# lazear/sage

Measured on AMD Instinct MI355X. Metric: spectra/sec (whole node), fragment-index search-and-score, human tryptic narrow search, higher is better.
Workload: dtype f32

## Files before the change

sage_amd/csrc/core.h:

```cpp
#pragma once
#include <stdint.h>

#if defined(__HIPCC__)
#define SAGE_HD __host__ __device__ __forceinline__
#else
#define SAGE_HD inline
#endif

namespace sagecore {

constexpr float PROTON = 1.0072764f;
constexpr float NEUTRON = 1.00335f;

struct Tol {
    int kind;
    float lo, hi;
};

SAGE_HD void tol_bounds(const Tol& t, float center, float& out_lo, float& out_hi) {
    if (t.kind == 0) {
        float dlo = center * t.lo / 1000000.0f;
        float dhi = center * t.hi / 1000000.0f;
        out_lo = center + dlo;
        out_hi = center + dhi;
// ... 537 lines not shown
constexpr uint32_t PLUT_BINS = 256;
SAGE_HD float peak_lut_width(float top) {
    uint32_t bits;
    __builtin_memcpy(&bits, &top, 4);
    const uint32_t e = (bits >> 23) & 0xFFu;
    uint32_t we = (bits >> 31) || e < 134u ? 127u : e - 7u;
    we = we > 227u ? 227u : we;
    const uint32_t wb = we << 23;
    float w;
    __builtin_memcpy(&w, &wb, 4);
    return w;
}
SAGE_HD float pow2_reciprocal(float w) {
    uint32_t bits;
    __builtin_memcpy(&bits, &w, 4);
    bits = 0x7F000000u - bits;
    float r;
    __builtin_memcpy(&r, &bits, 4);
    return r;
}
SAGE_HD uint32_t peak_lut_entry(const float* pm, uint32_t P, uint32_t b, float w) {
    if (b == 0) return 0;
    const int32_t edge = order_key((float)b * w);
    uint32_t lo = 0, hi = P;
    while (lo < hi) {
        const uint32_t mid = (lo + hi) >> 1;
        if (order_key(pm[mid]) < edge) lo = mid + 1; else hi = mid;
    }
    return lo;
}
SAGE_HD int select_peak_lut(const float* pm, const float* pi, uint32_t P, const uint32_t* plut, float inv_w, float lo, float hi) {
    float fb = __builtin_floorf(lo * inv_w);
    fb = fb > 0.0f ? fb : 0.0f;
    const uint32_t bin = fb < (float)(PLUT_BINS - 1) ? (uint32_t)fb : PLUT_BINS - 1;
    int best = -1;
    float max_int = 0.0f;
    for (uint32_t a = plut[bin]; a < P; a += 2) {
        const float m0 = pm[a], m1 = pm[a + 1 < P ? a + 1 : a];
        if (m0 >= lo && m0 <= hi) {
            const float it = pi[a];
            if (it >= max_int) { max_int = it; best = (int)a; }
        }
        if (a + 1 < P && m1 >= lo && m1 <= hi) {
            const float it = pi[a + 1];
            if (it >= max_int) { max_int = it; best = (int)(a + 1); }
        }
        if (m0 > hi || m1 > hi || !(hi == hi)) break;
    }
    return best;
}

SAGE_HD uint32_t wpp_step(uint32_t span) { return span / 65u + 1u; }

#ifndef SAGE_PBM_LOG2_BITS
#define SAGE_PBM_LOG2_BITS 15
#endif
#ifndef SAGE_PBM_LOG2_INV_W
#define SAGE_PBM_LOG2_INV_W 4
#endif
constexpr uint32_t PBM_BITS = 1u << SAGE_PBM_LOG2_BITS, PBM_WORDS = PBM_BITS / 32;
constexpr float PBM_INV_W = (float)(1u << SAGE_PBM_LOG2_INV_W);
constexpr float PBM_MAX_D = 4.0f;
SAGE_HD uint32_t pbm_index(float ion) {
#if defined(__HIP_DEVICE_COMPILE__)
    const float f = ion * PBM_INV_W;
    uint32_t x;
    asm("v_cvt_u32_f32 %0, %1" : "=v"(x) : "v"(f));
    return x;
#else
    const float f = ion * PBM_INV_W;
    return f >= 4294967296.0f ? 0xFFFFFFFFu : f > 0.0f ? (uint32_t)f : 0u;
#endif
}
SAGE_HD uint32_t pbm_bin_c1(uint32_t x) { return x & (PBM_BITS - 1u); }
SAGE_HD uint32_t pbm_bin_c2(uint32_t x) { return (x >> 1) & (PBM_BITS - 1u); }
SAGE_HD uint32_t pbm_bin_c3(uint32_t x) { return (uint32_t)(((uint64_t)x * 0xAAAAAAABull) >> 33) & (PBM_BITS - 1u); }
struct PbmReach {
    float a, b;
};
SAGE_HD PbmReach pbm_reach_of(const Tol& t) {
    const float tmax = __builtin_fmaxf(__builtin_fabsf(t.lo), __builtin_fabsf(t.hi));
    const float rel = t.kind == 0 ? tmax * 1.0e-6f : t.kind == 1 ? tmax * 1.0e-2f : 0.0f;
    PbmReach r{-1.0f, 0.0f};
    if (!(tmax == tmax) || !(tmax < 1.0e30f) || !(rel < 0.25f)) return r;
    r.a = (rel / (1.0f - rel)) * 1.0002f + (1.0f / 1048576.0f);
    r.b = (t.kind == 2 ? tmax * 1.0002f : 0.0f) + (1.0f / 1048576.0f);
    return r;
}
SAGE_HD bool pbm_peak_reach(const PbmReach& r, float m, float& D) {
    D = __builtin_fmaf(m, r.a, r.b);
    return r.a >= 0.0f && m >= 0.0f && m < 8388608.0f && D <= PBM_MAX_D;
}
SAGE_HD void pbm_peak_span(float m, float D, uint32_t& b0, uint32_t& b1) {
    const float f0 = (m - D) * PBM_INV_W, f1 = (m + D) * PBM_INV_W;
    b0 = f0 > 0.0f ? (uint32_t)f0 : 0u;
    b1 = f1 > 0.0f ? (uint32_t)f1 : 0u;
}

SAGE_HD uint32_t flat_octets(uint32_t n_here) { return (n_here + 7u) >> 3; }
SAGE_HD uint32_t flat_item_k(uint32_t t, uint32_t owner_start) { return t - owner_start; }
SAGE_HD uint64_t flat_item_base(uint64_t chunk_at, uint32_t owner_start) { return chunk_at - 8ull * owner_start; }
SAGE_HD uint64_t flat_item_ion(uint64_t item_base, uint32_t t) { return item_base + 8ull * t; }
SAGE_HD uint32_t flat_stride(uint32_t total) { return (total + 3u) & ~3u; }
SAGE_HD uint32_t flat_area_bytes(uint32_t total, uint32_t ncharges) { return flat_stride(total) * ncharges + 12u; }
#ifndef SAGE_FLAT_MARGIN
#define SAGE_FLAT_MARGIN 1
// ... 15 lines not shown
```

sage_amd/csrc/kernels.hip:

```cpp
#include <hip/hip_runtime.h>

#include <type_traits>

#include "crlog.h"
#include "device_types.h"

using namespace sagecore;

namespace sagehip {

namespace {

#ifndef SAGE_PRELIM_WAVES
#define SAGE_PRELIM_WAVES 5
#endif
#ifndef SAGE_RESCORE_WAVES
#define SAGE_RESCORE_WAVES 5
#endif
#ifndef SAGE_NARROW_WAVES
#define SAGE_NARROW_WAVES 5
#endif
#ifndef SAGE_PROBE_PER_LANE
#define SAGE_PROBE_PER_LANE 2
#endif
#ifndef SAGE_PROBE_CELLS
#define SAGE_PROBE_CELLS 4
#endif
#ifndef SAGE_TILE8_CELLS
#define SAGE_TILE8_CELLS 2
#endif
#ifndef SAGE_MARK_BLOCKS8
#define SAGE_MARK_BLOCKS8 96
#endif
#ifndef SAGE_MARK_BLOCKS16
#define SAGE_MARK_BLOCKS16 40
#endif
#ifndef SAGE_COOP_MIN_HITS
#define SAGE_COOP_MIN_HITS 12
#endif
#ifndef SAGE_COOP_MAX_LANES
#define SAGE_COOP_MAX_LANES 2
#endif
#ifndef SAGE_CNT_MODE
#define SAGE_CNT_MODE 0
#endif
#ifndef SAGE_SCAN_SKIP
#define SAGE_SCAN_SKIP 1
#endif
#if SAGE_NARROW_WAVES
#define SAGE_NARROW_WAVES_ATTR __attribute__((amdgpu_waves_per_eu(SAGE_NARROW_WAVES, SAGE_NARROW_WAVES)))
#else
#define SAGE_NARROW_WAVES_ATTR
#endif
#if SAGE_PRELIM_WAVES
#define SAGE_PRELIM_WAVES_ATTR __attribute__((amdgpu_waves_per_eu(SAGE_PRELIM_WAVES, SAGE_PRELIM_WAVES)))
#else
#define SAGE_PRELIM_WAVES_ATTR
#endif
#if SAGE_RESCORE_WAVES
#define SAGE_RESCORE_WAVES_ATTR __attribute__((amdgpu_waves_per_eu(SAGE_RESCORE_WAVES, SAGE_RESCORE_WAVES)))
#else
#define SAGE_RESCORE_WAVES_ATTR
#endif

constexpr uint32_t WAVE = 64;
constexpr uint32_t NO_WINDOW = 0xFFFFFFFFu;
constexpr uint32_t FAST_TIE_WORDS = PBM_WORDS + PLUT_BINS;
constexpr uint32_t CNT_ROW_HEADER = 4;
constexpr uint32_t PROBE_BATCH_WORDS = SAGE_PROBE_PER_LANE * 64;
constexpr uint32_t PROBE_TCS_WORDS = PROBE_BATCH_WORDS <= 64 ? 64 : PROBE_BATCH_WORDS <= 128 ? 128 : PROBE_BATCH_WORDS <= 256 ? 256 : 512;
constexpr uint32_t PROBE_TABLE_WORDS = 4 * PROBE_BATCH_WORDS + PROBE_TCS_WORDS;

enum { DBG_PRUNE_CAND = 0, DBG_PRUNE_ITEMS = 1, DBG_PRUNE_EARLY = 2, DBG_PRUNE_MIXED = 3 };
enum { DBG_FILTER_FLAT_CHUNKS = 4, DBG_FILTER_FLAT_TRIPS = 5, DBG_FILTER_FLAT_WOULD = 6, DBG_FILTER_LANE_TRIPS = 7 };
enum { DBG_HEAVY_CHUNKS = 8, DBG_HEAVY_ITEMS = 9 };
enum { DBG_HEAVY_ONE_TRIP = 10, DBG_HEAVY_PER_CHARGE = 11 };
enum { DBG_NARROW_LUT = 26, DBG_NARROW_CELLS = 27, DBG_RESCORE = 28, DBG_TILE_LUT = 29, DBG_TILE_CELLS = 30, DBG_TILE_CAND = 31 };
struct PhaseClock {
    unsigned long long* slot;
    long long t;
    __device__ __forceinline__ void bytes(int which, unsigned long long n) {
        if (slot) atomicAdd(&slot[which - row_base], n);
    }
    int row_base;
    unsigned long long* prune;
    uint32_t pruned_here;
    __device__ __forceinline__ void pruned(uint64_t lanes, uint32_t items) {
        if (slot && lanes) {
            pruned_here += (uint32_t)__popcll(lanes);
            if ((threadIdx.x & 63u) == 0) {
                atomicAdd(&prune[DBG_PRUNE_CAND], (unsigned long long)__popcll(lanes));
                atomicAdd(&prune[DBG_PRUNE_ITEMS], (unsigned long long)items);
            }
        }
    }
    __device__ __forceinline__ void filter_trips(bool flat, uint32_t flat_trips, uint32_t lane_trips) {
        if (slot && (threadIdx.x & 63u) == 0) {
            if (flat) {
                atomicAdd(&prune[DBG_FILTER_FLAT_CHUNKS], 1ull);
                atomicAdd(&prune[DBG_FILTER_FLAT_TRIPS], (unsigned long long)flat_trips);
                atomicAdd(&prune[DBG_FILTER_FLAT_WOULD], (unsigned long long)lane_trips);
            } else {
                atomicAdd(&prune[DBG_FILTER_LANE_TRIPS], (unsigned long long)lane_trips);
            }
        }
    }
    __device__ __forceinline__ void heavy(uint32_t items) {
        if (slot && (threadIdx.x & 63u) == 0) {
            atomicAdd(&prune[DBG_HEAVY_CHUNKS], 1ull);
            atomicAdd(&prune[DBG_HEAVY_ITEMS], (unsigned long long)items);
        }
    }
    __device__ __forceinline__ void heavy_route(bool one_trip) {
        if (slot && (threadIdx.x & 63u) == 0) atomicAdd(&prune[one_trip ? DBG_HEAVY_ONE_TRIP : DBG_HEAVY_PER_CHARGE], 1ull);
    }
    __device__ __forceinline__ void prune_outcome(bool left_early, bool any_pass) {
        if (slot && (threadIdx.x & 63u) == 0) {
            if (left_early) atomicAdd(&prune[DBG_PRUNE_EARLY], 1ull);
            else if (any_pass && pruned_here) atomicAdd(&prune[DBG_PRUNE_MIXED], 1ull);
        }
        pruned_here = 0;
    }
// ... 315 lines not shown
            uint32_t rank = 0;
            if (i < nst)
                for (uint32_t j = 0; j < nst; j++) {
                    const uint64_t o = c.items[j];
                    rank += (o > keep_v[q]) || (o == keep_v[q] && j < i);
                }
            keep_r[q] = i < nst ? rank : 0xFFFFFFFFu;
        }
        wave_sync();
#pragma unroll
        for (uint32_t q = 0; q < 4; q++)
            if (keep_r[q] < k) c.items[keep_r[q]] = keep_v[q];
        for (uint32_t i = nst + lane; i < k; i += WAVE) c.items[i] = PRESCORE_EMPTY;
        wave_sync();
    }
    c.stored = k;
    c.len = k;
}

__device__ __forceinline__ void lh_build(uint64_t* a, uint32_t k) {
    wave_sync();
    if (lane_id() == 0) heap_build(a, k);
    wave_sync();
}
__device__ __forceinline__ void lh_offer_batch(uint64_t* a, uint32_t k, uint64_t v, bool has) {
    if (!k) return;
    uint64_t mask = __ballot(has && v > a[0]);
    if (!mask) return;
    while (mask) {
        const uint32_t bit = (uint32_t)__ffsll((long long)mask) - 1;
        mask &= mask - 1;
        const uint64_t o = lane_value(v, bit);
        if (lane_id() == 0) heap_offer(a, k, o);
    }
    wave_sync();
}
__device__ __forceinline__ void ulist_trim_big(UList& c, uint32_t report_psms) {
    const uint32_t lane = lane_id();
    const uint32_t k = trim_k(c.len, report_psms);
    if (c.len > k) {
        lh_build(c.items, k);
        for (uint32_t base = k; base < c.stored; base += WAVE) {
            const bool has = base + lane < c.stored;
            lh_offer_batch(c.items, k, has ? c.items[base + lane] : 0ull, has);
        }
    }
    c.stored = k;
    c.len = k;
}

struct PrelimLds {
    float* win_lo;
    float* win_hi;
    uint64_t* listA;
    uint64_t* listB;
    uint64_t* heap;
    uint32_t* ptab;
    uint32_t* cnt;
};

__device__ __forceinline__ PrelimLds carve_prelim(unsigned char* smem, const DevScorer& sc, const DevBatchView& b, unsigned char* big = nullptr) {
    PrelimLds l;
    size_t off = 0;
    const bool fold = sc.min_isotope_err != sc.max_isotope_err;
    if (big) {
        l.listA = (uint64_t*)big;
        l.listB = l.listA + (fold ? (size_t)sc.list_cap : 0);
        l.heap = l.listB + sc.list_cap;
    } else {
        l.listA = (uint64_t*)(smem + off); off += fold ? (size_t)sc.list_cap * 8 : 0;
        l.listB = (uint64_t*)(smem + off); off += (size_t)sc.list_cap * 8;
        l.heap = (uint64_t*)(smem + off); off += (size_t)sc.kmax * 8;
    }
    const size_t win = b.probe ? (size_t)b.pcap * 4 : (size_t)b.fzcap * b.pcap * 4;
    l.win_lo = (float*)(smem + off); off += win;
    l.win_hi = (float*)(smem + off); off += b.probe ? 0 : win;
    off = (off + 3) & ~(size_t)3;
    l.ptab = (uint32_t*)(smem + off); off += b.probe ? (size_t)PROBE_TABLE_WORDS * 4 : 0;
    l.cnt = (uint32_t*)(smem + off);
    return l;
}

__host__ __device__ inline size_t prelim_big_bytes(const DevScorer& sc) {
    const bool fold = sc.min_isotope_err != sc.max_isotope_err;
    return (size_t)sc.list_cap * (fold ? 16 : 8) + (size_t)sc.kmax * 8;
}
__host__ __device__ inline size_t prelim_layout_bytes(const DevScorer& sc, const DevBatchView& b, bool huge = false) {
    size_t n = (huge ? 0 : prelim_big_bytes(sc)) +
               (b.probe ? (size_t)b.pcap * 4 + 4 + (size_t)PROBE_TABLE_WORDS * 4 : (size_t)b.fzcap * b.pcap * 8);
    n += ((size_t)sc.wcap / 2 + 1) * 4;
    return (n + 15) & ~(size_t)15;
}

struct SpecInfo {
    uint64_t p0;
    uint32_t P, z0, z1, nfz_max;
    float mzp;
    Tol iso_tol;
    Window win;
    bool has_win;
};
__device__ __forceinline__ SpecInfo load_spec(const DevScorer& sc, const DevBatchView& b, uint32_t spec) {
    SpecInfo s;
    s.win = Window{0u, 0u, 0u, 0u};
    s.has_win = false;
    s.p0 = uni64(b.peak_off[spec]);
    s.P = (uint32_t)(uni64(b.peak_off[spec + 1]) - s.p0);
    const uint32_t zraw = uni(b.precursor_charge[spec]);
    if (sc.wide_window || zraw == 0 || sc.override_precursor_charge) {
        s.z0 = sc.min_precursor_charge;
        s.z1 = sc.max_precursor_charge;
    } else {
        s.z0 = s.z1 = zraw;
    }
    s.nfz_max = 0;
    for (uint32_t z = s.z0; z <= s.z1; z++) {
        const uint32_t m = max_fragment_charge(sc.max_fragment_charge, z) - 1;
        s.nfz_max = m > s.nfz_max ? m : s.nfz_max;
    }
    if (s.nfz_max > b.fzcap) s.nfz_max = b.fzcap;
    s.mzp = unif(b.precursor_mz[spec]) - PROTON;
    s.iso_tol.kind = 2;
    s.iso_tol.lo = -2.4f;
    s.iso_tol.hi = 2.4f;
    if (b.isolation_lo && b.isolation_hi) {
        const float a = unif(b.isolation_lo[spec]), c = unif(b.isolation_hi[spec]);
        if (a == a && c == c) {
            s.iso_tol.lo = a;
            s.iso_tol.hi = c;
            if (b.iso_kind) s.iso_tol.kind = (int32_t)uni(b.iso_kind[spec]);
        }
    }
    return s;
}

__device__ __forceinline__ SpecInfo load_spec_sched(const DevScorer& sc, const DevBatchView& b, uint32_t pos, uint32_t& spec) {
    const uint4* __restrict__ rec = b.sched + (size_t)b.sched_stride * pos;
    const uint4 r0 = rec[0], r1 = rec[1];
    uint4 r2 = make_uint4(NO_WINDOW, 0u, 0u, 0u);
    if (b.sched_win) r2 = rec[2];
    spec = uni(r0.x);
    SpecInfo s;
// ... 119 lines not shown
    }
    wave_sync();
    ulist_append(target, lane < nsel ? sel[lane] : PRESCORE_EMPTY, k, kmax);
    wave_sync();
    return true;
}

constexpr uint32_t PROBE_PER_LANE = SAGE_PROBE_PER_LANE;
constexpr uint32_t PROBE_BATCH = PROBE_PER_LANE * 64;
constexpr uint32_t PROBE_CELLS = SAGE_PROBE_CELLS;
static_assert(PROBE_BATCH == PROBE_BATCH_WORDS && PROBE_BATCH <= 512, "the run table's layout (carve_prelim) is the kernel's");
static_assert(PROBE_TCS_WORDS - PROBE_BATCH <= WAVE, "one sentinel per lane pads the run starts");
struct PrelimKernargs {
    DevDbView db;
    DevScorer sc;
    DevBatchView b;
    DevWork w;
};
#define SAGE_LOAD_TOL(t) Tol{(t).kind, (t).lo, (t).hi}
template <class K>
struct ArgRef {
    const DevDbView& db_;
    const DevScorer& sc_;
    const DevBatchView& b_;
    __device__ __forceinline__ ArgRef(const DevDbView& d, const DevScorer& s, const DevBatchView& b) : db_(d), sc_(s), b_(b) {}
    __device__ __forceinline__ void refresh() {}
    __device__ __forceinline__ const DevDbView& db() const { return db_; }
    __device__ __forceinline__ const DevScorer& sc() const { return sc_; }
    __device__ __forceinline__ const DevBatchView& b() const { return b_; }
};
template <>
struct ArgRef<PrelimKernargs> {
    typedef const __attribute__((address_space(4))) PrelimKernargs* Segment;
    Segment ka;
    __device__ __forceinline__ ArgRef(const DevDbView&, const DevScorer&, const DevBatchView&)
        : ka((Segment)__builtin_amdgcn_kernarg_segment_ptr()) {}
    __device__ __forceinline__ void refresh() {
        ka = (Segment)__builtin_amdgcn_kernarg_segment_ptr();
        asm volatile("" : "+s"(ka));
    }
    __device__ __forceinline__ const __attribute__((address_space(4))) DevDbView& db() const { return ka->db; }
    __device__ __forceinline__ const __attribute__((address_space(4))) DevScorer& sc() const { return ka->sc; }
    __device__ __forceinline__ const __attribute__((address_space(4))) DevBatchView& b() const { return ka->b; }
};

struct PrelimResult {
    uint32_t stored;
    uint32_t matched, scored;
    bool ok;
    bool deferred;
    bool untrimmed;
    uint32_t q_left, q_potential;
};
template <bool PROBE, bool BIGK = false, class KA = void, class PC>
__device__ __forceinline__ PrelimResult prelim_spectrum(const DevDbView& db_, const DevScorer& sc_, const DevBatchView& b_, const PrelimLds& L,
                                                        const SpecInfo& si, const bool exact, PC& pc) {
    const uint32_t lane = lane_id();
    ArgRef<KA> av(db_, sc_, b_);
    av.refresh();
    Counters cnt;
    cnt.p = L.cnt;
    PrelimResult res{0u, 0u, 0u, true, false, true, 0u, 0u};
    {
        const uint32_t P = si.P, nfz_max = si.nfz_max;
        const float* __restrict__ masses = av.b().masses + si.p0;
        const uint32_t pcap = av.b().pcap;
        const Tol ftol0 = SAGE_LOAD_TOL(av.sc().fragment_tol);

        float pk0 = 0.f, pk1 = 0.f, pk2 = 0.f;
        Window q_first{0u, 0u, 0u, 0u};
        bool have_first = false;
        int iso_first = 0;
        if (PROBE) {
            if (lane < P) pk0 = masses[lane];
            if (lane + WAVE < P) pk1 = masses[lane + WAVE];
            if (lane + 2 * WAVE < P) pk2 = masses[lane + 2 * WAVE];
        }
        if (si.z0 <= si.z1) {
            const bool fold0 = av.sc().min_isotope_err != av.sc().max_isotope_err;
            iso_first = fold0 ? av.sc().min_isotope_err : 0;
            if (si.has_win && !(av.sc().dbg_flags & 65536u)) {
                q_first = si.win;
                have_first = true;
            } else if (PROBE) {
                const float precursor_mass = si.mzp * (float)si.z0;
                const Tol ptol = av.sc().wide_window ? tol_scaled(si.iso_tol, (float)si.z0) : SAGE_LOAD_TOL(av.sc().precursor_tol);
                const float center = precursor_mass - (float)iso_first * NEUTRON;
                q_first = query_window<true>(av.db().pep_mono, av.db().np, ptol, center, av.db().pep_lut, av.db().pep_lut_bins, av.db().pep_lut_inv_w);
                have_first = true;
            }
        }
        if (PROBE) {
            if (lane < P) L.win_lo[lane] = pk0;
            if (lane + WAVE < P) L.win_lo[lane + WAVE] = pk1;
            if (lane + 2 * WAVE < P) L.win_lo[lane + 2 * WAVE] = pk2;
        }
        for (uint32_t i = PROBE ? lane + 3 * WAVE : lane; i < P; i += WAVE) {
            const float m = masses[i];
            if (PROBE) {
                L.win_lo[i] = m;
                continue;
            }
            for (uint32_t fz = 1; fz <= nfz_max; fz++) {
                float lo, hi;
                tol_bounds(ftol0, m * (float)fz, lo, hi);
                L.win_lo[(size_t)(fz - 1) * pcap + i] = lo;
                L.win_hi[(size_t)(fz - 1) * pcap + i] = hi;
            }
        }
        __syncthreads();
        if (pc.slot && lane == 0) pc.bytes(DBG_NARROW_CELLS, 4ull * P);
        bool sorted_ok = true;
        uint32_t ptop = 0;
        if (!PROBE) {
            bool mono_ok = true;
            for (uint32_t fz = 0; fz < nfz_max; fz++) {
                const float* wl = L.win_lo + (size_t)fz * pcap;
                const float* wh = L.win_hi + (size_t)fz * pcap;
                for (uint32_t i = lane; i < P; i += WAVE) {
                    mono_ok = mono_ok && (wl[i] <= wh[i]);
                    if (i > 0) mono_ok = mono_ok && (wl[i - 1] <= wl[i]) && (wh[i - 1] <= wh[i]);
                }
            }
            sorted_ok = __ballot(!mono_ok) == 0ull;
            ptop = pow2_floor(P);
        }
        pc.mark(0);

        av.refresh();
        const bool fold = av.sc().min_isotope_err != av.sc().max_isotope_err;
        const int isoA = fold ? av.sc().min_isotope_err : 0, isoB = fold ? av.sc().max_isotope_err : 0;

        UList A, B;
        A.items = L.listA; A.cap = fold ? av.sc().list_cap : 0; A.stored = 0; A.len = 0; A.ok = true;
        B.items = L.listB; B.cap = av.sc().list_cap; B.stored = 0; B.len = 0; B.ok = true;
        bool deferred = false;
        uint32_t tot_matched = 0, tot_scored = 0;

        for (uint32_t z = si.z0; z <= si.z1 && !deferred; z++) {
            av.refresh();
            const uint32_t nfz = max_fragment_charge(av.sc().max_fragment_charge, z) - 1;
            const float precursor_mass = si.mzp * (float)z;
            const Tol ptol = av.sc().wide_window ? tol_scaled(si.iso_tol, (float)z) : SAGE_LOAD_TOL(av.sc().precursor_tol);
            if (fold) { A.stored = 0; A.len = 0; }
            for (int iso = isoA; iso <= isoB && !deferred; iso++) {
                const float center = precursor_mass - (float)iso * NEUTRON;
                av.refresh();
                const Window q = have_first && z == si.z0 && iso == iso_first
                                     ? q_first
                                     : query_window<true>(av.db().pep_mono, av.db().np, ptol, center, av.db().pep_lut, av.db().pep_lut_bins, av.db().pep_lut_inv_w);
// ... 59 lines not shown
                    const uint32_t t0 = q.first >> tile2_shift, t1 = (q.end - 1) >> tile2_shift;
                    const uint32_t nprobe = P * nfz;
                    uint32_t* const tp0 = L.ptab;
                    uint32_t* const tp1 = L.ptab + PROBE_BATCH;
                    uint32_t* const tcs = L.ptab + 4 * PROBE_BATCH;
                    float* const tlo = (float*)(L.ptab + 2 * PROBE_BATCH);
                    float* const thi = (float*)(L.ptab + 3 * PROBE_BATCH);
                    if (PROBE_TCS_WORDS > PROBE_BATCH && lane < PROBE_TCS_WORDS - PROBE_BATCH) tcs[PROBE_BATCH + lane] = NO_WINDOW;
                    const bool sym_ppm = (av.sc().tol_mode & TOL_SYM) != 0u && ftol.kind == 0;
                    auto window_of = [&](uint32_t pr, float& flo, float& fhi) {
                        flo = 1.0f; fhi = 0.0f;
                        const bool has = pr < nprobe;
                        float center = 0.f;
                        if (has) {
                            const uint32_t fz = pr / P, i = pr - fz * P;
                            center = L.win_lo[i] * (float)(fz + 1);
                        }
                        if (sym_ppm) {
                            const float x = center * ftol.hi, ax = __builtin_fabsf(x);
                            float d;
                            if (__ballot(has && !(ax >= FAST_DIV_LO && ax <= FAST_DIV_HI)) == 0ull) d = div_1e6_fast(x);
                            else d = x / 1000000.0f;
                            if (has) { flo = center + -d; fhi = center + d; }
                        } else if (has) {
                            tol_bounds(ftol, center, flo, fhi);
                        }
                    };
                    for (uint32_t t = t0; t <= t1; t++) {
                        const LutWord* __restrict__ l1 = tm2_l1 + (size_t)t * lut2_words;
                        uint32_t np0[PROBE_PER_LANE], np1[PROBE_PER_LANE];
                        float nlo[PROBE_PER_LANE], nhi[PROBE_PER_LANE];
                        auto issue = [&](uint32_t pbase) {
                            uint32_t icl[PROBE_PER_LANE], ich[PROBE_PER_LANE];
                            LutWord wa[PROBE_PER_LANE], wb[PROBE_PER_LANE];
#pragma unroll
                            for (uint32_t i = 0; i < PROBE_PER_LANE; i++) {
                                window_of(pbase + i * WAVE + lane, nlo[i], nhi[i]);
                                lut_cells(nlo[i], nhi[i], lut2_scale, lut2_stride, icl[i], ich[i]);
                                wa[i] = l1[icl[i] >> 5];
                                wb[i] = l1[ich[i] >> 5];
                            }
#pragma unroll
                            for (uint32_t i = 0; i < PROBE_PER_LANE; i++) {
                                const uint32_t r0 = lut_rank(wa[i], icl[i]), r1 = lut_rank(wb[i], ich[i]);
                                np0[i] = np1[i] = 0;
                                if (r1 > r0) {
                                    np0[i] = tm2_pos[r0];
                                    np1[i] = tm2_pos[r1];
                                }
                            }
                        };
                        issue(0);
                        for (uint32_t pbase = 0; pbase < nprobe; pbase += PROBE_BATCH) {
                            uint32_t rp0[PROBE_PER_LANE], rp1[PROBE_PER_LANE];
#pragma unroll
                            for (uint32_t i = 0; i < PROBE_PER_LANE; i++) {
                                rp0[i] = np0[i]; rp1[i] = np1[i];
                                tlo[lane * PROBE_PER_LANE + i] = nlo[i];
                                thi[lane * PROBE_PER_LANE + i] = nhi[i];
                            }
                            if (pbase + PROBE_BATCH < nprobe) issue(pbase + PROBE_BATCH);
                            uint32_t tot = 0;
#pragma unroll
                            for (uint32_t i = 0; i < PROBE_PER_LANE; i++) tot += rp1[i] > rp0[i] ? ((rp1[i] - 1) >> 1) - (rp0[i] >> 1) + 1 : 0;
                            const uint32_t incl = wave_incl_scan_dpp(tot);
                            uint32_t run = incl - tot;
#pragma unroll
                            for (uint32_t i = 0; i < PROBE_PER_LANE; i++) {
                                tp0[lane * PROBE_PER_LANE + i] = rp0[i];
                                tp1[lane * PROBE_PER_LANE + i] = rp1[i];
                                tcs[lane * PROBE_PER_LANE + i] = run;
                                run += rp1[i] > rp0[i] ? ((rp1[i] - 1) >> 1) - (rp0[i] >> 1) + 1 : 0;
                            }
                            const uint32_t n_cells = (uint32_t)__builtin_amdgcn_readlane((int)incl, 63);
                            if (pc.slot) {
                                uint32_t nonempty = 0;
#pragma unroll
                                for (uint32_t i = 0; i < PROBE_PER_LANE; i++) nonempty += (uint32_t)__popcll(__ballot(rp1[i] > rp0[i]));
                                if (lane == 0) {
                                    const uint32_t nw = nprobe - pbase < PROBE_BATCH ? nprobe - pbase : PROBE_BATCH;
                                    pc.bytes(DBG_NARROW_LUT, 16ull * nw + 8ull * nonempty);
                                    pc.bytes(DBG_NARROW_CELLS, 16ull * n_cells);
                                }
                            }
                            wave_sync();
                            for (uint32_t cb = 0; cb < n_cells; cb += WAVE * PROBE_CELLS) {
                                uint4 e[PROBE_CELLS];
                                uint32_t eq[PROBE_CELLS], ej[PROBE_CELLS];
#pragma unroll
                                for (uint32_t c = 0; c < PROBE_CELLS; c++) {
                                    const uint32_t k = cb + c * WAVE + lane;
                                    e[c] = make_uint4(0u, 0u, 0u, 0u);
                                    eq[c] = NO_WINDOW;
                                    ej[c] = 0;
                                    if (k < n_cells) {
                                        uint32_t a = 0;
#pragma unroll
                                        for (uint32_t step = PROBE_TCS_WORDS / 2; step; step >>= 1) a += (tcs[a + step] <= k) ? step : 0;
                                        eq[c] = a;
                                        ej[c] = ((tp0[a] >> 1) + (k - tcs[a])) << 1;
                                        e[c] = frag2[ej[c] >> 1];
                                    }
                                }
#pragma unroll
                                for (uint32_t c = 0; c < PROBE_CELLS; c++) {
                                    if (eq[c] == NO_WINDOW) continue;
                                    const uint32_t a = eq[c];
                                    const float lo = tlo[a], hi = thi[a];
                                    const uint32_t p0 = tp0[a], p1 = tp1[a], j = ej[c];
                                    const float mz0 = __uint_as_float(e[c].y), mz1 = __uint_as_float(e[c].w);
                                    if (j >= p0 && j < p1 && mz0 >= lo && mz0 <= hi && e[c].x >= q.first && e[c].x < q.end) { cnt.add(e[c].x - left, 1); acc++; }
                                    if (j + 1 < p1 && mz1 >= lo && mz1 <= hi && e[c].z >= q.first && e[c].z < q.end) { cnt.add(e[c].z - left, 1); acc++; }
                                }
                            }
                            wave_sync();
                        }
                    }
                }
                const uint32_t matched = wave_sum(acc);
                __syncthreads();
                pc.mark(2);
                av.refresh();
                const uint32_t kmax = av.sc().kmax, report_psms = av.sc().report_psms;
                res.q_left = left;
                res.q_potential = potential;
                tot_matched += matched;
                UList& target = fold ? A : B;
                if (matched == 0) {
                    ulist_append_empties(target, potential, kmax);
                    continue;
                }
                const uint32_t k = trim_k(potential, report_psms);
                uint32_t scored = 0;
                if (potential <= k) {
                    for (uint32_t base = 0; base < potential; base += WAVE) {
                        const uint32_t i = base + lane;
                        const uint32_t c = i < potential ? cnt.get(i) : 0;
                        scored += (uint32_t)__popcll(__ballot(c > 0));
                        const uint32_t nvalid = potential - base < WAVE ? potential - base : WAVE;
// ... 14 lines not shown
                        const uint32_t c = i < potential ? cnt.get(i) : 0;
                        scored += (uint32_t)__popcll(__ballot(c > 0));
                        lh_offer_batch(hp, k, pack_prescore(c, left + i, z, iso), c > 0);
                    }
                    for (uint32_t base = 0; base < k; base += WAVE)
                        ulist_append(target, base + lane < k ? hp[base + lane] : PRESCORE_EMPTY, k - base < WAVE ? k - base : WAVE, kmax);
                } else if (!exact && fast_select(L, cnt, potential, k, left, z, iso, kmax, target, scored)) {
                    res.untrimmed = false;
                } else {
                    res.untrimmed = false;
                    scored = 0;
                    Heap32 hp;
                    {
                        const uint32_t c = lane < k ? cnt.get(lane) : 0;
                        wh32_init(hp, c ? (c << 16) | lane : 0u, k);
                        scored += (uint32_t)__popcll(__ballot(c > 0));
                    }
                    wh32_build(hp, k);
                    for (uint32_t base = k; base < potential; base += WAVE) {
                        const uint32_t i = base + lane;
                        const uint32_t c = i < potential ? cnt.get(i) : 0;
                        const uint32_t v = (c << 16) | i;
                        uint64_t mask = __ballot(c > 0 && c >= (wh32_get(hp, 0) >> 16));
                        scored += (uint32_t)__popcll(__ballot(c > 0));
                        if (pc.slot && lane == 0) atomicAdd(&pc.slot[5], (unsigned long long)__popcll(mask));
                        while (mask) {
                            const uint32_t bit = (uint32_t)__ffsll((long long)mask) - 1;
                            mask &= mask - 1;
                            wh32_offer(hp, k, (uint32_t)__builtin_amdgcn_readlane((int)v, (int)__builtin_amdgcn_readfirstlane(bit)));
                        }
                    }
                    const uint32_t h = hp.h;
                    ulist_append(target, h ? pack_prescore(h >> 16, left + (h & 0xFFFFu), z, iso) : PRESCORE_EMPTY, k, kmax);
                }
                tot_scored += scored;
                __syncthreads();
                pc.mark(3);
            }
            if (fold && !deferred) {
                av.refresh();
                const uint32_t kmax = av.sc().kmax, report_psms = av.sc().report_psms;
                if (A.len > trim_k(A.len, report_psms)) res.untrimmed = false;
                if (BIGK) ulist_trim_big(A, report_psms);
                else ulist_trim(A, report_psms, exact || av.sc().list_cap > 4 * WAVE);
                __syncthreads();
                for (uint32_t base = 0; base < A.stored; base += WAVE) {
                    const uint64_t v = base + lane < A.stored ? A.items[base + lane] : PRESCORE_EMPTY;
                    const uint32_t nvalid = A.stored - base < WAVE ? A.stored - base : WAVE;
                    ulist_append(B, v, nvalid, kmax);
                }
                __syncthreads();
            }
        }
        if (deferred) {
            res.deferred = true;
            return res;
        }
        av.refresh();
        const uint32_t report_psms = av.sc().report_psms;
        if (B.len > trim_k(B.len, report_psms)) res.untrimmed = false;
        if (BIGK) ulist_trim_big(B, report_psms);
        else ulist_trim(B, report_psms, exact || av.sc().list_cap > 4 * WAVE);
        __syncthreads();
        res.stored = B.stored;
        res.matched = tot_matched;
        res.scored = tot_scored;
        res.ok = A.ok && B.ok;
    }
    return res;
}

template <bool PROBE, bool PROF, bool BIGK = false, bool HUGE = false>
__global__ __launch_bounds__(64) SAGE_PRELIM_WAVES_ATTR void prelim_kernel(PrelimKernargs A) {
    const DevDbView& db = A.db;
    const DevScorer& sc = A.sc;
    const DevBatchView& b = A.b;
    const DevWork& w = A.w;
    typedef typename std::conditional<PROF, PhaseClock, NoClock>::type Clock;
    extern __shared__ __align__(16) unsigned char smem[];
    const uint32_t lane = lane_id();
    const PrelimLds L = carve_prelim(smem, sc, b, BIGK && HUGE ? w.hugebuf + (size_t)blockIdx.x * w.huge_stride : nullptr);

    uint32_t n_batch = b.n;
    if (b.n_dev) {
        const uint32_t nd = uni(*b.n_dev);
        n_batch = nd < n_batch ? nd : n_batch;
    }
    for (uint32_t blk = blockIdx.x; blk < n_batch; blk += gridDim.x) {
        const uint32_t pos = xcd_position(blk, n_batch, sc.xcd_chunk);
        uint32_t spec = b.sched ? 0u : b.order ? uni(b.order[pos]) : pos;
        __syncthreads();
        Clock pc;
        pc.start((sc.dbg_flags & 512u) && !sc.exact ? nullptr : w.dbg, blk, 0);
        const SpecInfo si = b.sched ? load_spec_sched(sc, b, pos, spec) : load_spec(sc, b, spec);
        const PrelimResult r = prelim_spectrum<PROBE, BIGK, PrelimKernargs>(db, sc, b, L, si, sc.exact != 0, pc);
        typedef const __attribute__((address_space(4))) PrelimKernargs* Segment;
        Segment ka = (Segment)__builtin_amdgcn_kernarg_segment_ptr();
        asm volatile("" : "+s"(ka));
        uint32_t* const w_cnt_store = ka->w.cnt_store;
        if (!BIGK && w_cnt_store) {
            const bool keep = !r.deferred && si.z0 == si.z1 && ka->sc.min_isotope_err == ka->sc.max_isotope_err;
            uint32_t* __restrict__ row = w_cnt_store + (size_t)pos * ka->w.cnt_stride;
            if (keep && SAGE_CNT_MODE != 1)
                for (uint32_t i = lane; i < (r.q_potential + 1) / 2; i += WAVE) row[CNT_ROW_HEADER + i] = L.cnt[i];
            if (lane == 0 && SAGE_CNT_MODE != 2) {
                row[0] = keep ? r.q_left : 0u;
                row[1] = keep ? r.q_potential : 0u;
            }
        }
        uint64_t* const w_hand = BIGK ? nullptr : ka->w.hand;
        if (w_hand) {
            const uint32_t st = r.deferred ? (uint32_t)ST_DEFERRED : r.ok ? (r.untrimmed ? (uint32_t)ST_OK_ORDERED : (uint32_t)ST_OK) : (uint32_t)ST_OVERFLOW;
            const uint32_t stored = r.deferred ? 0u : (r.stored < HAND_LIST_MAX ? r.stored : HAND_LIST_MAX);
            uint64_t v = lane < stored ? L.listB[lane] : PRESCORE_EMPTY;
            if (lane == HAND_HEAD_WORD) v = (uint64_t)stored << 32 | st;
            if (lane == HAND_TOTALS_WORD) v = r.deferred ? 0ull : (uint64_t)r.scored << 32 | r.matched;
            w_hand[(size_t)pos * HAND_ROW_WORDS + lane] = v;
        }
        if (r.deferred) {
            if (lane == 0) {
                ka->w.status[spec] = ST_DEFERRED;
                if (!ka->w.queue_later) {
                    const uint32_t it = atomicAdd(ka->w.n_deferred + CTR_QUEUED, 1u);
                    ka->w.queue[it] = spec;
                    if (!ka->w.reuse) ka->w.item_of[spec] = it;
                }
            }
            continue;
        }
        if (lane == 0 && !r.ok) atomicAdd(ka->w.n_deferred + CTR_LIST_OVERFLOW, 1u);
        if (!w_hand) {
            if (lane == 0) {
                ka->w.status[spec] = r.ok ? (r.untrimmed ? ST_OK_ORDERED : ST_OK) : ST_OVERFLOW;
                ka->w.cand_len[spec] = r.stored;
                ka->w.totals[2 * spec] = r.matched;
                ka->w.totals[2 * spec + 1] = r.scored;
            }
            uint64_t* __restrict__ dst = ka->w.cand + (size_t)spec * ka->sc.kmax;
            for (uint32_t i = lane; i < r.stored; i += WAVE) dst[i] = L.listB[i];
        }
        pc.mark(4);
    }
}

__global__ __launch_bounds__(256) void queue_kernel(DevScorer sc, DevBatchView b, DevWork w) {
    uint32_t n_batch = b.n;
    if (b.n_dev) {
        const uint32_t nd = *b.n_dev;
// ... 2980 lines not shown
                o->n_site_items = ns;
#pragma unroll
                for (uint32_t j = 0; j < DEPTHS / 2; j++) {
                    o->a[j] = na[2 * j] | (na[2 * j + 1] << 16);
                    o->b[j] = nb[2 * j] | (nb[2 * j + 1] << 16);
                }
            }
        }
        if (sc.chimera && r + 1 < ranks) localise_next_rank(db, sc, feats[slot0 + r].peptide_idx, fcharge, pm, pi, rm, rm2, rk, P);
    }
}

}

size_t prelim_lds_bytes(const DevScorer& sc, const DevBatchView& b, bool huge) { return prelim_layout_bytes(sc, b, huge); }
size_t huge_stride_bytes(const DevScorer& sc) {
    const uint32_t ks = ((sc.kmax + 63u) / 64u) * 64u;
    size_t n = prelim_big_bytes(sc);
    n = n > assemble_lds_bytes(sc) ? n : assemble_lds_bytes(sc);
    n = n > rescore_big_bytes(true, ks) ? n : rescore_big_bytes(true, ks);
    n = n > (size_t)ks * 8 ? n : (size_t)ks * 8;
    return (n + 255) & ~(size_t)255;
}
size_t tile_lds_bytes(const DevDbView& db, const DevScorer&, const DevBatchView& b, bool cnt8, bool wing) {
    return tile_lds_layout(db.tile_shift, b, nullptr, nullptr, cnt8, wing);
}
size_t assemble_lds_bytes(const DevScorer& sc) {
    const bool fold = sc.min_isotope_err != sc.max_isotope_err;
    return ((size_t)sc.list_cap * (fold ? 16 : 8) + 15) & ~(size_t)15;
}
uint32_t fast_tie_lds_words() { return FAST_TIE_WORDS; }
uint32_t huge_grid() { return HUGE_GRID; }
int bigk_kernel_prepare(size_t max_lds_bytes) {
    for (const void* f : {(const void*)prelim_kernel<true, false, true>, (const void*)prelim_kernel<false, false, true>,
                          (const void*)prelim_kernel<true, false, true, true>, (const void*)prelim_kernel<false, false, true, true>,
                          (const void*)rescore_big_kernel<false, false>, (const void*)rescore_big_kernel<true, false>,
                          (const void*)rescore_big_kernel<false, true>, (const void*)rescore_big_kernel<true, true>,
                          (const void*)tile_assemble_kernel<true>, (const void*)tile_assemble_kernel<true, true>,
                          (const void*)tile_replay_big_kernel<false>, (const void*)tile_replay_big_kernel<true>}) {
        const hipError_t e = hipFuncSetAttribute(f, hipFuncAttributeMaxDynamicSharedMemorySize, (int)max_lds_bytes);
        if (e != hipSuccess) return (int)e;
    }
    return (int)hipSuccess;
}
int tile_kernel_prepare(size_t max_lds_bytes) {
    for (const void* f : {(const void*)tile_count_kernel, (const void*)tile_count8_kernel, (const void*)tile_count_wing_kernel}) {
        const hipError_t e = hipFuncSetAttribute(f, hipFuncAttributeMaxDynamicSharedMemorySize, (int)max_lds_bytes);
        if (e != hipSuccess) return (int)e;
    }
    return (int)hipSuccess;
}
int spectrum_kernel_prepare(size_t max_lds_bytes) {
    for (const void* f : {(const void*)prelim_kernel<true, true>, (const void*)prelim_kernel<true, false>, (const void*)prelim_kernel<false, true>,
                          (const void*)prelim_kernel<false, false>, (const void*)rescore_kernel<true, true>, (const void*)rescore_kernel<false, false>,
                          (const void*)rescore_kernel<false, false, true>, (const void*)rescore_kernel<false, true>,
                          (const void*)rescore_kernel<true, true, false, false>, (const void*)rescore_kernel<false, false, false, false>,
                          (const void*)rescore_kernel<false, false, true, false>, (const void*)rescore_kernel<false, true, false, false>,
                          (const void*)rescore_kernel<true, true, false, false, true>, (const void*)rescore_kernel<false, false, false, false, true>,
                          (const void*)rescore_kernel<false, false, true, false, true>,
                          (const void*)narrow_kernel<true, true>, (const void*)narrow_kernel<true, false>,
                          (const void*)narrow_kernel<false, true>, (const void*)narrow_kernel<false, false>, (const void*)annotate_kernel,
                          (const void*)candidates_kernel, (const void*)depth_counts_kernel, (const void*)site_counts_kernel}) {
        const hipError_t e = hipFuncSetAttribute(f, hipFuncAttributeMaxDynamicSharedMemorySize, (int)max_lds_bytes);
        if (e != hipSuccess) return (int)e;
        hipFuncAttributes at;
        if (hipFuncGetAttributes(&at, f) == hipSuccess && at.sharedSizeBytes != 0) return (int)hipErrorInvalidConfiguration;
    }
#ifdef SAGE_HIP_EXPERIMENTS
    for (const void* f : {(const void*)search_kernel<true, true>, (const void*)search_kernel<true, false>, (const void*)search_kernel<false, true>,
                          (const void*)search_kernel<false, false>}) {
        const hipError_t e = hipFuncSetAttribute(f, hipFuncAttributeMaxDynamicSharedMemorySize, (int)max_lds_bytes);
        if (e != hipSuccess) return (int)e;
    }
#endif
    return (int)hipSuccess;
}
uint32_t queries_per_spectrum(const DevScorer& sc) {
    const uint32_t n_iso = sc.min_isotope_err != sc.max_isotope_err ? (uint32_t)(sc.max_isotope_err - sc.min_isotope_err) + 1 : 1;
    return (sc.max_precursor_charge - sc.min_precursor_charge + 1) * n_iso;
}
size_t rescore_lds_bytes(const DevScorer& sc, const DevBatchView& b, uint32_t, bool quick, bool huge) {
    if (sc.big_path)
        return ((rescore_scratch_bytes(false) + 15) & ~(size_t)15) + rescore_fixed_bytes(sc, b) +
               (huge ? 0 : rescore_big_bytes(quick, ((sc.kmax + 63u) / 64u) * 64u));
    return ((rescore_scratch_bytes(quick) + 15) & ~(size_t)15) + rescore_fixed_bytes(sc, b);
}
size_t narrow_lds_bytes(const DevScorer& sc, const DevBatchView& b) { return narrow_scratch_bytes(sc, b) + rescore_fixed_bytes(sc, b); }

#ifdef SAGE_HIP_EXPERIMENTS
size_t search_lds_bytes(const DevScorer& sc, const DevBatchView& b) {
    const size_t a = prelim_layout_bytes(sc, b), r = rescore_lds_bytes(sc, b, 0, false);
    return a > r ? a : r;
}
void launch_search(const DevDbView& db, const DevScorer& sc, const DevBatchView& b, const DevWork& w, const double* lnfact_table,
                   uint32_t lnfact_n, SageFeature* out, uint32_t* out_count, void* stream) {
    if (b.n == 0) return;
    auto k = b.probe ? (w.dbg ? search_kernel<true, true> : search_kernel<true, false>)
                     : (w.dbg ? search_kernel<false, true> : search_kernel<false, false>);
    hipLaunchKernelGGL(k, dim3(2 * search_slots(b.n)), dim3(64), search_lds_bytes(sc, b), (hipStream_t)stream, db, sc, b, w, lnfact_table,
                       lnfact_n, out, out_count);
}
#else
size_t search_lds_bytes(const DevScorer&, const DevBatchView&) { return 0; }
void launch_search(const DevDbView&, const DevScorer&, const DevBatchView&, const DevWork&, const double*, uint32_t, SageFeature*, uint32_t*, void*) {}
#endif
void launch_narrow(const DevDbView& db, const DevScorer& sc, const DevBatchView& b, const DevWork& w, const double* lnfact_table,
                   uint32_t lnfact_n, SageFeature* out, uint32_t* out_count, void* stream) {
    if (b.n == 0) return;
    auto k = b.probe ? (w.dbg ? narrow_kernel<true, true> : narrow_kernel<true, false>)
                     : (w.dbg ? narrow_kernel<false, true> : narrow_kernel<false, false>);
    const uint32_t grid = b.n_dev ? (b.n < RETRY_GRID_CAP ? b.n : RETRY_GRID_CAP) : b.n;
    const RescoreKernargs args{db, sc, b, w, lnfact_table, lnfact_n, out, out_count, nullptr};
    hipLaunchKernelGGL(k, dim3(grid), dim3(64), narrow_lds_bytes(sc, b), (hipStream_t)stream, args);
}
void launch_prelim(const DevDbView& db, const DevScorer& sc, const DevBatchView& b, const DevWork& w, void* stream) {
    if (b.n == 0) return;
    auto k = b.probe ? (w.dbg ? prelim_kernel<true, true> : prelim_kernel<true, false>)
                     : (w.dbg ? prelim_kernel<false, true> : prelim_kernel<false, false>);
    if (sc.big_path) k = b.probe ? prelim_kernel<true, false, true> : prelim_kernel<false, false, true>;
    if (sc.big_path && w.hugebuf) k = b.probe ? prelim_kernel<true, false, true, true> : prelim_kernel<false, false, true, true>;
    uint32_t grid = sc.big_path && w.hugebuf && b.n > HUGE_GRID ? HUGE_GRID : b.n;
    static const uint32_t grid_cap = [] { const char* e = getenv("SAGE_HIP_PRELIM_GRID"); return e ? (uint32_t)strtoul(e, nullptr, 10) & ~7u : 0u; }();
    if (grid_cap && grid > grid_cap) grid = grid_cap;
    hipLaunchKernelGGL(k, dim3(grid), dim3(64), prelim_lds_bytes(sc, b, sc.big_path && w.hugebuf), (hipStream_t)stream, PrelimKernargs{db, sc, b, w});
}
void launch_queue(const DevScorer& sc, const DevBatchView& b, const DevWork& w, void* stream) {
    if (b.n == 0) return;
    const uint32_t blocks = (b.n + 255u) / 256u;
    hipLaunchKernelGGL(queue_kernel, dim3(blocks < 4096u ? blocks : 4096u), dim3(256), 0, (hipStream_t)stream, sc, b, w);
}
void launch_prelim_tile(const DevDbView& db, const DevScorer& sc, const DevBatchView& b, const DevWork& w, void* stream,
                        const SideStream* side) {
    if (b.n == 0 || w.tile_blocks == 0) return;
    const bool fold = sc.min_isotope_err != sc.max_isotope_err;
    if (w.winbuf)
        hipLaunchKernelGGL(tile_count_wing_kernel, dim3(w.tile_blocks < b.n ? w.tile_blocks : b.n), dim3(TILE_THREADS),
                           tile_lds_bytes(db, sc, b, false, true), (hipStream_t)stream, TileParams{db, sc, b, w});
    else if (w.cnt8)
        hipLaunchKernelGGL(tile_count8_kernel, dim3(w.tile_blocks < b.n ? w.tile_blocks : b.n), dim3(TILE_THREADS),
                           tile_lds_bytes(db, sc, b, true), (hipStream_t)stream, TileParams{db, sc, b, w});
    else
        hipLaunchKernelGGL(tile_count_kernel, dim3(w.tile_blocks < b.n ? w.tile_blocks : b.n), dim3(TILE_THREADS),
                           tile_lds_bytes(db, sc, b, false), (hipStream_t)stream, TileParams{db, sc, b, w});
    if (hipPeekAtLastError() != hipSuccess) return;
    const uint64_t nq = (uint64_t)b.n * w.qmax;
    const uint32_t grid_cap = sc.big_path && w.hugebuf ? HUGE_GRID : TILE_GRID_CAP;
    auto capped = [grid_cap](uint64_t blocks) { return (uint32_t)(blocks < grid_cap ? blocks : grid_cap); };
    const size_t assemble_lds = sc.big_path && w.hugebuf ? 0 : assemble_lds_bytes(sc);
    (void)fold;
    if (sc.big_path) {
        if (w.hugebuf) {
            hipLaunchKernelGGL(tile_replay_big_kernel<true>, dim3(capped(nq)), dim3(64), WAVE * 4, (hipStream_t)stream, sc, w);
            hipLaunchKernelGGL((tile_assemble_kernel<true, true>), dim3(capped(b.n)), dim3(64), assemble_lds, (hipStream_t)stream, sc, b, w);
        } else {
            hipLaunchKernelGGL(tile_replay_big_kernel<false>, dim3(capped(nq)), dim3(64), (size_t)w.kstride * 8 + WAVE * 4, (hipStream_t)stream, sc, w);
            hipLaunchKernelGGL(tile_assemble_kernel<true>, dim3(capped(b.n)), dim3(64), assemble_lds, (hipStream_t)stream, sc, b, w);
        }
        return;
    }
    uint64_t wave_max = w.replay_split;
    if (!sc.exact && (wave_max & 0xFFFFFFFFull)) wave_max |= 0xFFFFFFFFull;
    const bool both = (wave_max & 0xFFFFFFFFull) != 0xFFFFFFFFull && (sc.exact || !(wave_max & 0xFFFFFFFFull));
    const bool select = !sc.exact;
    hipStream_t side_stream = (hipStream_t)stream;
    if ((select || both) && side) {
        side_stream = (hipStream_t)side->stream;
        if (hipEventRecord((hipEvent_t)side->fork, (hipStream_t)stream) != hipSuccess) return;
        if (hipStreamWaitEvent(side_stream, (hipEvent_t)side->fork, 0) != hipSuccess) return;
    }
    if (select) hipLaunchKernelGGL(tile_select_kernel, dim3(capped(nq)), dim3(64), 0, side_stream, sc, w);
    if (both) hipLaunchKernelGGL(tile_replay_kernel, dim3(capped((nq + 63) / 64)), dim3(64), 0, side_stream, sc, w, wave_max);
    hipLaunchKernelGGL(tile_replay_wave_kernel, dim3(capped(nq)), dim3(64), 0, (hipStream_t)stream, sc, w, wave_max);
    if ((select || both) && side) {
        if (hipEventRecord((hipEvent_t)side->join, side_stream) != hipSuccess) return;
        if (hipStreamWaitEvent((hipStream_t)stream, (hipEvent_t)side->join, 0) != hipSuccess) return;
    }
    hipLaunchKernelGGL(tile_assemble_kernel<false>, dim3(capped(b.n)), dim3(64), assemble_lds, (hipStream_t)stream, sc, b, w);
// ... 137 lines not shown
```

Baseline: 162.6 million.

## Group prelim probe blocks into XCD-strided turns with optional next-spectrum LDS prefetch

For probe-mode, non-big prelim launches, each workgroup now processes several spectra (turns) spaced by the XCD count instead of one block per spectrum, so the grid shrinks. An optional look-ahead variant, gated by a debug flag bit, uses global_load_lds to stage the next spectrum's peak masses into a second LDS window during the current spectrum's probe loop, then swaps the window buffers. The goal is to amortize workgroup launch and setup cost and to hide the peak-load latency of the next spectrum. The cost is less parallelism, possible load imbalance within turns, and extra LDS for the look-ahead path. The env-var grid cap has been removed.

```diff
diff --git a/sage_amd/csrc/core.h b/sage_amd/csrc/core.h
--- a/sage_amd/csrc/core.h
+++ b/sage_amd/csrc/core.h
@@ -613,6 +613,13 @@
 
 SAGE_HD uint32_t wpp_step(uint32_t span) { return span / 65u + 1u; }
 
+constexpr uint32_t TURN_XCDS = 8;
+SAGE_HD uint32_t turn_first_block(uint32_t g, uint32_t turns) { return (g / TURN_XCDS) * turns * TURN_XCDS + g % TURN_XCDS; }
+SAGE_HD uint32_t turn_grid(uint32_t n, uint32_t turns) {
+    const uint32_t rows = n / TURN_XCDS + (n % TURN_XCDS != 0u ? 1u : 0u);
+    return (rows / turns + (rows % turns != 0u ? 1u : 0u)) * TURN_XCDS;
+}
+
 #ifndef SAGE_PBM_LOG2_BITS
 #define SAGE_PBM_LOG2_BITS 15
 #endif
diff --git a/sage_amd/csrc/kernels.hip b/sage_amd/csrc/kernels.hip
--- a/sage_amd/csrc/kernels.hip
+++ b/sage_amd/csrc/kernels.hip
@@ -13,6 +13,9 @@
 
 #ifndef SAGE_PRELIM_WAVES
 #define SAGE_PRELIM_WAVES 5
+#endif
+#ifndef SAGE_PRELIM_TURNS
+#define SAGE_PRELIM_TURNS 2
 #endif
 #ifndef SAGE_RESCORE_WAVES
 #define SAGE_RESCORE_WAVES 5
@@ -68,6 +71,7 @@
 constexpr uint32_t FAST_TIE_WORDS = PBM_WORDS + PLUT_BINS;
 constexpr uint32_t CNT_ROW_HEADER = 4;
 constexpr uint32_t PROBE_BATCH_WORDS = SAGE_PROBE_PER_LANE * 64;
+constexpr size_t PRELIM_AHEAD_LDS_MAX = 160u * 1024u / 20u;
 constexpr uint32_t PROBE_TCS_WORDS = PROBE_BATCH_WORDS <= 64 ? 64 : PROBE_BATCH_WORDS <= 128 ? 128 : PROBE_BATCH_WORDS <= 256 ? 256 : 512;
 constexpr uint32_t PROBE_TABLE_WORDS = 4 * PROBE_BATCH_WORDS + PROBE_TCS_WORDS;
 
@@ -489,6 +493,7 @@
 struct PrelimLds {
     float* win_lo;
     float* win_hi;
+    float* win_nx;
     uint64_t* listA;
     uint64_t* listB;
     uint64_t* heap;
@@ -496,7 +501,8 @@
     uint32_t* cnt;
 };
 
-__device__ __forceinline__ PrelimLds carve_prelim(unsigned char* smem, const DevScorer& sc, const DevBatchView& b, unsigned char* big = nullptr) {
+__device__ __forceinline__ PrelimLds carve_prelim(unsigned char* smem, const DevScorer& sc, const DevBatchView& b, unsigned char* big = nullptr,
+                                                 const bool ahead = false) {
     PrelimLds l;
     size_t off = 0;
     const bool fold = sc.min_isotope_err != sc.max_isotope_err;
@@ -512,6 +518,7 @@
     const size_t win = b.probe ? (size_t)b.pcap * 4 : (size_t)b.fzcap * b.pcap * 4;
     l.win_lo = (float*)(smem + off); off += win;
     l.win_hi = (float*)(smem + off); off += b.probe ? 0 : win;
+    l.win_nx = (float*)(smem + off); off += ahead ? win : 0;
     off = (off + 3) & ~(size_t)3;
     l.ptab = (uint32_t*)(smem + off); off += b.probe ? (size_t)PROBE_TABLE_WORDS * 4 : 0;
     l.cnt = (uint32_t*)(smem + off);
@@ -522,9 +529,9 @@
     const bool fold = sc.min_isotope_err != sc.max_isotope_err;
     return (size_t)sc.list_cap * (fold ? 16 : 8) + (size_t)sc.kmax * 8;
 }
-__host__ __device__ inline size_t prelim_layout_bytes(const DevScorer& sc, const DevBatchView& b, bool huge = false) {
+__host__ __device__ inline size_t prelim_layout_bytes(const DevScorer& sc, const DevBatchView& b, bool huge = false, bool ahead = false) {
     size_t n = (huge ? 0 : prelim_big_bytes(sc)) +
-               (b.probe ? (size_t)b.pcap * 4 + 4 + (size_t)PROBE_TABLE_WORDS * 4 : (size_t)b.fzcap * b.pcap * 8);
+               (b.probe ? (size_t)b.pcap * (ahead ? 8 : 4) + 4 + (size_t)PROBE_TABLE_WORDS * 4 : (size_t)b.fzcap * b.pcap * 8);
     n += ((size_t)sc.wcap / 2 + 1) * 4;
     return (n + 15) & ~(size_t)15;
 }
@@ -750,10 +757,25 @@
     bool untrimmed;
     uint32_t q_left, q_potential;
 };
-template <bool PROBE, bool BIGK = false, class KA = void, class PC>
+constexpr uint32_t AHEAD_STAGED = 0xFFFFFFFDu, AHEAD_DONE = 0xFFFFFFFEu;
+struct StageAhead {
+    static constexpr bool on = true;
+    uint32_t next;
+    bool staged_in, staged_out;
+};
+struct NoAhead {
+    static constexpr bool on = false;
+    static constexpr uint32_t next = NO_WINDOW;
+    static constexpr bool staged_in = false;
+    bool staged_out;
+};
+template <bool PROBE, bool BIGK = false, class KA = void, class PC, class AH>
 __device__ __forceinline__ PrelimResult prelim_spectrum(const DevDbView& db_, const DevScorer& sc_, const DevBatchView& b_, const PrelimLds& L,
-                                                        const SpecInfo& si, const bool exact, PC& pc) {
+                                                        const SpecInfo& si, const bool exact, PC& pc, AH& ah) {
     const uint32_t lane = lane_id();
+    const bool staged = AH::on && PROBE && ah.staged_in;
+    uint32_t ahead_pos = AH::on && PROBE ? ah.next : NO_WINDOW;
+    ah.staged_out = false;
     ArgRef<KA> av(db_, sc_, b_);
     av.refresh();
     Counters cnt;
@@ -769,7 +791,7 @@
         Window q_first{0u, 0u, 0u, 0u};
         bool have_first = false;
         int iso_first = 0;
-        if (PROBE) {
+        if (PROBE && !staged) {
             if (lane < P) pk0 = masses[lane];
             if (lane + WAVE < P) pk1 = masses[lane + WAVE];
             if (lane + 2 * WAVE < P) pk2 = masses[lane + 2 * WAVE];
@@ -788,12 +810,12 @@
                 have_first = true;
             }
         }
-        if (PROBE) {
+        if (PROBE && !staged) {
             if (lane < P) L.win_lo[lane] = pk0;
             if (lane + WAVE < P) L.win_lo[lane + WAVE] = pk1;
             if (lane + 2 * WAVE < P) L.win_lo[lane + 2 * WAVE] = pk2;
         }
-        for (uint32_t i = PROBE ? lane + 3 * WAVE : lane; i < P; i += WAVE) {
+        for (uint32_t i = PROBE ? (staged ? P : lane + 3 * WAVE) : lane; i < P; i += WAVE) {
             const float m = masses[i];
             if (PROBE) {
                 L.win_lo[i] = m;
@@ -959,6 +981,13 @@
                         };
                         issue(0);
                         for (uint32_t pbase = 0; pbase < nprobe; pbase += PROBE_BATCH) {
+                            const bool stage_now = AH::on && ahead_pos < AHEAD_STAGED;
+                            uint32_t nx_P = 0, nx_lo = 0, nx_hi = 0;
+                            if (stage_now) {
+                                typedef const __attribute__((address_space(4))) uint32_t* RecWords;
+                                const RecWords nr = (RecWords)(av.b().sched + (size_t)av.b().sched_stride * ahead_pos);
+                                nx_P = nr[1]; nx_lo = nr[2]; nx_hi = nr[3];
+                            }
                             uint32_t rp0[PROBE_PER_LANE], rp1[PROBE_PER_LANE];
 #pragma unroll
                             for (uint32_t i = 0; i < PROBE_PER_LANE; i++) {
@@ -992,6 +1021,18 @@
                             }
                             wave_sync();
                             for (uint32_t cb = 0; cb < n_cells; cb += WAVE * PROBE_CELLS) {
+                                if (AH::on) __builtin_amdgcn_s_waitcnt(0x0F70);
+                                if (stage_now && cb == 0) {
+                                    ahead_pos = AHEAD_DONE;
+                                    if (nx_P <= av.b().pcap) {
+                                        const float* __restrict__ src = av.b().masses + (((uint64_t)nx_hi << 32) | nx_lo);
+                                        for (uint32_t base = 0; base < nx_P; base += WAVE)
+                                            if (base + lane < nx_P)
+                                                __builtin_amdgcn_global_load_lds((const __attribute__((address_space(1))) void*)(src + base + lane),
+                                                                                 (__attribute__((address_space(3))) void*)(L.win_nx + base), 4, 0, 0);
+                                        ahead_pos = AHEAD_STAGED;
+                                    }
+                                }
                                 uint4 e[PROBE_CELLS];
                                 uint32_t eq[PROBE_CELLS], ej[PROBE_CELLS];
 #pragma unroll
@@ -1112,6 +1153,7 @@
                 __syncthreads();
             }
         }
+        ah.staged_out = AH::on && ahead_pos == AHEAD_STAGED;
         if (deferred) {
             res.deferred = true;
             return res;
@@ -1129,8 +1171,14 @@
     }
     return res;
 }
-
-template <bool PROBE, bool PROF, bool BIGK = false, bool HUGE = false>
+template <bool PROBE, bool BIGK = false, class KA = void, class PC>
+__device__ __forceinline__ PrelimResult prelim_spectrum(const DevDbView& db, const DevScorer& sc, const DevBatchView& b, const PrelimLds& L,
+                                                        const SpecInfo& si, const bool exact, PC& pc) {
+    NoAhead none{false};
+    return prelim_spectrum<PROBE, BIGK, KA>(db, sc, b, L, si, exact, pc, none);
+}
+
+template <bool PROBE, bool PROF, bool BIGK = false, bool HUGE = false, bool AHEAD = false>
 __global__ __launch_bounds__(64) SAGE_PRELIM_WAVES_ATTR void prelim_kernel(PrelimKernargs A) {
     const DevDbView& db = A.db;
     const DevScorer& sc = A.sc;
@@ -1139,21 +1187,43 @@
     typedef typename std::conditional<PROF, PhaseClock, NoClock>::type Clock;
     extern __shared__ __align__(16) unsigned char smem[];
     const uint32_t lane = lane_id();
-    const PrelimLds L = carve_prelim(smem, sc, b, BIGK && HUGE ? w.hugebuf + (size_t)blockIdx.x * w.huge_stride : nullptr);
+    static_assert(!AHEAD || (PROBE && !BIGK), "the look-ahead belongs to the grouped turns of the probe instances");
+    PrelimLds L = carve_prelim(smem, sc, b, BIGK && HUGE ? w.hugebuf + (size_t)blockIdx.x * w.huge_stride : nullptr, AHEAD);
 
     uint32_t n_batch = b.n;
     if (b.n_dev) {
         const uint32_t nd = uni(*b.n_dev);
         n_batch = nd < n_batch ? nd : n_batch;
     }
-    for (uint32_t blk = blockIdx.x; blk < n_batch; blk += gridDim.x) {
-        const uint32_t pos = xcd_position(blk, n_batch, sc.xcd_chunk);
+    constexpr bool GROUPED = PROBE && !BIGK;
+    uint32_t blk = GROUPED ? turn_first_block(blockIdx.x, SAGE_PRELIM_TURNS) : blockIdx.x;
+    const uint32_t blk_step = GROUPED ? TURN_XCDS : gridDim.x;
+    const uint32_t blk_end = GROUPED && n_batch > blk && n_batch - blk > SAGE_PRELIM_TURNS * TURN_XCDS ? blk + SAGE_PRELIM_TURNS * TURN_XCDS : n_batch;
+    typename std::conditional<AHEAD, StageAhead, NoAhead>::type ah{};
+    ah.staged_out = false;
+    uint32_t pos_turn = AHEAD && blk < blk_end ? xcd_position(blk, n_batch, sc.xcd_chunk) : 0u, pos_next = 0u;
+    auto next_turn = [&] {
+        blk += blk_step;
+        if (AHEAD) {
+            pos_turn = pos_next;
+            float* const t = L.win_lo;
+            L.win_lo = L.win_nx;
+            L.win_nx = t;
+        }
+    };
+    for (; blk < blk_end; next_turn()) {
+        const uint32_t pos = AHEAD ? pos_turn : xcd_position(blk, n_batch, sc.xcd_chunk);
         uint32_t spec = b.sched ? 0u : b.order ? uni(b.order[pos]) : pos;
         __syncthreads();
         Clock pc;
         pc.start((sc.dbg_flags & 512u) && !sc.exact ? nullptr : w.dbg, blk, 0);
         const SpecInfo si = b.sched ? load_spec_sched(sc, b, pos, spec) : load_spec(sc, b, spec);
-        const PrelimResult r = prelim_spectrum<PROBE, BIGK, PrelimKernargs>(db, sc, b, L, si, sc.exact != 0, pc);
+        if constexpr (AHEAD) {
+            ah.staged_in = ah.staged_out;
+            const bool more = blk + blk_step < blk_end;
+            pos_next = more ? xcd_position(blk + blk_step, n_batch, sc.xcd_chunk) : 0u;
+            ah.next = b.sched && more ? pos_next : NO_WINDOW;        }
+        const PrelimResult r = prelim_spectrum<PROBE, BIGK, PrelimKernargs>(db, sc, b, L, si, sc.exact != 0, pc, ah);
         typedef const __attribute__((address_space(4))) PrelimKernargs* Segment;
         Segment ka = (Segment)__builtin_amdgcn_kernarg_segment_ptr();
         asm volatile("" : "+s"(ka));
@@ -4240,6 +4310,7 @@
 }
 int spectrum_kernel_prepare(size_t max_lds_bytes) {
     for (const void* f : {(const void*)prelim_kernel<true, true>, (const void*)prelim_kernel<true, false>, (const void*)prelim_kernel<false, true>,
+                          (const void*)prelim_kernel<true, true, false, false, true>, (const void*)prelim_kernel<true, false, false, false, true>,
                           (const void*)prelim_kernel<false, false>, (const void*)rescore_kernel<true, true>, (const void*)rescore_kernel<false, false>,
                           (const void*)rescore_kernel<false, false, true>, (const void*)rescore_kernel<false, true>,
                           (const void*)rescore_kernel<true, true, false, false>, (const void*)rescore_kernel<false, false, false, false>,
@@ -4308,9 +4379,16 @@
     if (sc.big_path) k = b.probe ? prelim_kernel<true, false, true> : prelim_kernel<false, false, true>;
     if (sc.big_path && w.hugebuf) k = b.probe ? prelim_kernel<true, false, true, true> : prelim_kernel<false, false, true, true>;
     uint32_t grid = sc.big_path && w.hugebuf && b.n > HUGE_GRID ? HUGE_GRID : b.n;
-    static const uint32_t grid_cap = [] { const char* e = getenv("SAGE_HIP_PRELIM_GRID"); return e ? (uint32_t)strtoul(e, nullptr, 10) & ~7u : 0u; }();
-    if (grid_cap && grid > grid_cap) grid = grid_cap;
-    hipLaunchKernelGGL(k, dim3(grid), dim3(64), prelim_lds_bytes(sc, b, sc.big_path && w.hugebuf), (hipStream_t)stream, PrelimKernargs{db, sc, b, w});
+    size_t lds = prelim_lds_bytes(sc, b, sc.big_path && w.hugebuf);
+    if (b.probe && !sc.big_path) {
+        grid = turn_grid(b.n, SAGE_PRELIM_TURNS);
+        const size_t lds_ahead = prelim_layout_bytes(sc, b, false, true);
+        if (b.sched && (sc.dbg_flags & 524288u) && lds_ahead <= PRELIM_AHEAD_LDS_MAX) {
+            k = w.dbg ? prelim_kernel<true, true, false, false, true> : prelim_kernel<true, false, false, false, true>;
+            lds = lds_ahead;
+        }
+    }
+    hipLaunchKernelGGL(k, dim3(grid), dim3(64), lds, (hipStream_t)stream, PrelimKernargs{db, sc, b, w});
 }
 void launch_queue(const DevScorer& sc, const DevBatchView& b, const DevWork& w, void* stream) {
     if (b.n == 0) return;
```

New measurement: 163.4 million, median of 6. No clear change (+0.5%).
